# shibatch/rectdetect

Hardware: AMD Instinct MI355X
Metric: 1920x1080 frames/sec (higher is better)
Workload: dtype u8/i32/f32 (bit-exact integer + IEEE f32 stencil path)

## Files before the change

### include/rectdetect_hip.h

```cpp
#ifndef RECTDETECT_HIP_H
#define RECTDETECT_HIP_H
#include <stddef.h>
#include <stdint.h>
#if defined(__cplusplus)
extern "C" {
#endif

const char *rd_version(void);
int rd_device_count(void);
void rd_select_device(int ordinal);
int rd_device_pci_bus_id(int ordinal, char *buf, int len);

void *rd_device_alloc(size_t bytes);
void rd_device_free(void *dptr);
void *rd_host_alloc(size_t bytes);
void rd_host_free(void *p);
void rd_upload(void *dptr, const void *host, size_t bytes);
void rd_download(void *host, const void *dptr, size_t bytes);

typedef struct rd_detector rd_detector;

rd_detector *rd_detector_create(int device, int iw, int ih, int nslots, int nworkers);
void rd_detector_destroy(rd_detector *d);

rd_detector *rd_polyline_detector_create(int device, int iw, int ih, int nslots, int strength_thre, float minerror, int size_thre);
void *rd_detector_poll_segments(rd_detector *d, int32_t *ids_out);

void rd_release_cached_streams(int device);

#define RD_FRAME_HOST 0
#define RD_FRAME_DEVICE 1
#define RD_FRAME_HOST_PINNED 2
long rd_detector_enqueue(rd_detector *d, const void *frame, int ws, int on_device);

#define RD_PIX_BGR  0
#define RD_PIX_RGB  1
#define RD_PIX_BGRA 2
#define RD_PIX_RGBA 3
#define RD_PIX_NV12 4
#define RD_PIX_I420 5
long rd_detector_enqueue_planes(rd_detector *d, int format, const void *const planes[3], const int pitches[3], int on_device);

void *rd_detector_poll(rd_detector *d, double tanAOV);

void rd_detector_set_aperture(rd_detector *d, double tanAOV);

void rd_detector_drain(rd_detector *d);

int rd_detector_last_segments(rd_detector *d, void *dst, int max_records);

long rd_detector_counter(rd_detector *d, int which);


size_t rd_detector_debug_plane(rd_detector *d, const char *name, void *dst, size_t max_bytes);

void *rd_postprocess_planes(const void *segs, const int32_t *boundary, const int32_t *table, int iw, int ih, double tanAOV);
void rd_probe_pixels(float x0, float y0, float x1, float y1, int iw, int ih, int32_t *out);


void rd_rect_quads(const void *rects, int n, double *quads_out);
double rd_rect_aspect(const void *rect);
void rd_rectify_coefficients(const double quad[8], double coef[8], int *status);

typedef struct rd_rectifier rd_rectifier;
rd_rectifier *rd_rectifier_create(int device, int pw, int ph, int max_quads, int njobs);
void rd_rectifier_destroy(rd_rectifier *r);

long rd_rectifier_enqueue(rd_rectifier *r, int format, const void *const planes[3], const int pitches[3], int iw, int ih, int on_device,
                          const double *quads, int n, void *out, int out_kind);
int rd_rectifier_wait(rd_rectifier *r, uint8_t *status_out);
long rd_detector_rectify_polled(rd_detector *d, rd_rectifier *r, const double *quads, int n, void *out, int out_kind);

int rd_synth_num_quads(int iw, int ih);
void rd_synth_frame(uint8_t *bgr, int iw, int ih, int ws, uint64_t seed, int t, int noise);

#if defined(__cplusplus)
}
#endif
#endif
```

### rectdetect_amd/__init__.py

```python
import ctypes
import os

import numpy as np

_HERE = os.path.dirname(os.path.abspath(__file__))
LIB_PATH = os.environ.get("RD_LIB_PATH") or os.path.join(_HERE, "librectdetect_hip.so")

RECT_DTYPE = np.dtype([("c2", "<f8", (4, 2)), ("c3", "<f8", (4, 3)), ("value", "<f8"), ("status", "<u4"), ("_pad", "<u4")])
LS_DTYPE = np.dtype([("x0", "<f4"), ("y0", "<f4"), ("x1", "<f4"), ("y1", "<f4"), ("startIndex", "<i4"), ("endIndex", "<i4"),
                     ("leftPtr", "<i4"), ("rightPtr", "<i4"), ("startCount", "<i4"), ("endCount", "<i4"), ("maxDist", "<i4"),
                     ("polyid", "<i4"), ("npix", "<i4"), ("level", "<i4")])
assert RECT_DTYPE.itemsize == 176 and LS_DTYPE.itemsize == 56

PIX_BGR, PIX_RGB, PIX_BGRA, PIX_RGBA, PIX_NV12, PIX_I420 = range(6)
PIX_NAMES = {PIX_BGR: "BGR", PIX_RGB: "RGB", PIX_BGRA: "BGRA", PIX_RGBA: "RGBA", PIX_NV12: "NV12", PIX_I420: "I420"}

CL_MEM_READ_WRITE = 1 << 0
CL_MEM_COPY_HOST_PTR = 1 << 5
CL_TRUE = 1

_lib = None


def lib():
# ... 428 lines not shown
            raise ValueError("rd_rectifier_enqueue: invalid arguments (format %r, pitches %r, %dx%d, %d quads, out %r)" % (fmt, pitch, iw, ih, n, out))
        return r

    def wait(self):
        status = np.zeros(self.max_quads, np.uint8)
        n = lib().rd_rectifier_wait(self.h, status.ctypes.data)
        if n < 0:
            raise RuntimeError("rd_rectifier_wait: no job in flight")
        return status[:n].copy()

    def rectify(self, frame_bgr, quads):
        a = np.asarray(frame_bgr, dtype=np.uint8)
        q, n = _quads_arg(quads)
        nbytes = max(n, 1) * self.ph * self.pw * 3
        p = lib().rd_host_alloc(nbytes)
        try:
            self.enqueue(PIX_BGR, a, None, a.shape[1], a.shape[0], q, p, out_pinned=True)
            self.wait()
            return np.frombuffer((ctypes.c_uint8 * nbytes).from_address(p), np.uint8)[:n * self.ph * self.pw * 3].reshape(n, self.ph, self.pw, 3).copy()
        finally:
            lib().rd_host_free(p)

    def close(self):
        if self.h:
            lib().rd_rectifier_destroy(self.h)
            self.h = None


def postprocess_planes(segs, boundary, table, iw, ih, tan_aov):
    segs = np.ascontiguousarray(segs)
    boundary = np.ascontiguousarray(boundary, dtype=np.int32)
    table = np.ascontiguousarray(table, dtype=np.int32)
    return _take_rects(lib().rd_postprocess_planes(segs.ctypes.data, boundary.ctypes.data, table.ctypes.data, iw, ih, float(tan_aov)))
```

### rectdetect_amd/csrc/rd_api.hip

```cpp
#include "rd_internal.h"
#include "rd_kernels.h"
#include "rd_poly_scratch.h"
#include "rectdetect_hip.h"
#include <stdio.h>
#include <stdlib.h>
#include <string.h>
#include <pthread.h>
#include <time.h>
#include <sched.h>

extern "C" {
#include "vec234.h"
#include "oclimgutil.h"
#include "oclpolyline.h"
#include "oclrect.h"
#include "rd_post.h"
}

using rdrt::dptr;
using rdrt::stream;

static const char *rd_env(const char *name) { const char *v = getenv(name); return (v && *v) ? v : NULL; }
static int rd_env_int(const char *name, int dflt) { const char *v = rd_env(name); return v ? atoi(v) : dflt; }
#ifdef RD_TUNING
// ... 1387 lines not shown
      if (!strcmp(name, "strong") || !strcmp(name, "mergemask") || !strcmp(name, "junction")) {
        return bit_plane_as_ints(d, tab[i].p, !strcmp(name, "junction"), dst, max_bytes);
      }
      if (!strcmp(name, "mask0")) {
        const size_t n = N * 4 <= max_bytes ? N : max_bytes / 4;
        float *tmp = (float *)malloc(n ? n * 4 : 4);
        if (!tmp) exitf(-1, "rd_detector_debug_plane: out of memory\n");
        RD_HIP(hipMemcpy(tmp, s->nms, n * 4, hipMemcpyDeviceToHost));
        for (size_t k = 0; k < n; k++) ((int *)dst)[k] = tmp[k] > 0.0f ? 1 : 0;
        free(tmp);
        return n * 4;
      }
      if (!strcmp(name, "edge500")) {
        const size_t n = N * 4 <= max_bytes ? N : max_bytes / 4;
        int8_t *tmp = (int8_t *)malloc(n ? n : 1);
        RD_HIP(hipMemcpy(tmp, tab[i].p, n, hipMemcpyDeviceToHost));
        for (size_t k = 0; k < n; k++) ((int *)dst)[k] = tmp[k];
        free(tmp);
        return n * 4;
      }
      RD_HIP(hipMemcpy(dst, tab[i].p, b, hipMemcpyDeviceToHost));
      if (!strcmp(name, "strsum") && s->prev_in) {
        const size_t n = b / 4;
        int8_t *tmp = (int8_t *)malloc(n ? n : 1);
        RD_HIP(hipMemcpy(tmp, s->prev_in, n, hipMemcpyDeviceToHost));
        for (size_t k = 0; k < n; k++) ((int *)dst)[k] += tmp[k];
        free(tmp);
      }
      return b;
    }
  return 0;
}

rd_detector *rd_polyline_detector_create(int device, int iw, int ih, int nslots, int strength_thre, float minerror, int size_thre) {
  if (iw < 16 || ih < 16 || (long long)iw * ih >= (1ll << 25) || nslots < 1 || device < 0 || strength_thre < 0 || !(minerror > 0.0f) || size_thre < 0) return NULL;
  if (rd_device_count() <= 0) exitf(-1, "rd_polyline_detector_create: no HIP device available - this library has no CPU path\n");
  if (device >= rd_device_count()) return NULL;
  rd_detector *d = detector_new(RD_KIND_POLY, device, iw, ih, nslots, 0);
  d->p_thre = strength_thre; d->p_minerror = minerror; d->p_size = size_thre;
  d->handoff_rec = RD_POLY_HANDOFF_DEFAULT;
  { const int h = rd_env_int("RD_POLY_HANDOFF", 0); if (h >= 2) d->handoff_rec = h; }
  detector_slots(d, 4);
  return d;
}

void *rd_detector_poll_segments(rd_detector *d, int32_t *ids_out) {
  if (!d || d->magic != MAGIC_RECT) exitf(-1, "rd_detector_poll_segments: bad handle\n");
  if (d->kind != RD_KIND_POLY) exitf(-1, "rd_detector_poll_segments: this is a rectangle detector (rd_detector_create) - its results come from rd_detector_poll\n");
  if (d->next_poll >= d->next_enqueue) exitf(-1, "rd_detector_poll_segments: nothing enqueued\n");
  RD_HIP(hipSetDevice(d->device));
  const int si = (int)(d->next_poll % d->nslots);
  Slot *s = &d->slots[si];
  const size_t N = (size_t)d->N;
  if (s->pending_dense) group_launch(d, si / d->zb * d->zb);
  RD_HIP(hipEventSynchronize(s->watch_done));
  const bool over = s->poly_mode == 1 && s->h_pack[25] != 0;
  if (s->poly_mode == 1) { if (over) { if (++d->overflow_streak >= 2) d->poly_overflows = 1; } else d->overflow_streak = 0; }
  if (!s->st_redo) s->st_redo = make_redo_stream();
  if (over || (d->force_redo & 1)) {
    rdk::polyline(s->st_redo, s->frame, 1, d->N * 16, 0, d->p_minerror, d->p_size, d->iw, d->ih, 0);
    rdk::polyline_handoff(s->st_redo, s->frame, 1, d->handoff_rec);
    rdrt::check_launch("polyline frame, multi-launch repeat");
    RD_HIP(hipStreamSynchronize(s->st_redo));
    d->n_redo++;
  }
  const int n = s->h_pack[64];
// ... 71 lines not shown
```

### rectdetect_amd/csrc/rd_k_rect.hip

```cpp
#include <stdlib.h>
#include "rd_device.h"
#include "rd_kernels.h"
#include "rd_tidy_tile.h"
#include "rd_poly_scratch.h"
#include "rd_post_core.h"
#include <atomic>

namespace {

using namespace rd;

inline int cdiv(int a, int b) { return (a + b - 1) / b; }
const dim3 block2(64, 4);
inline dim3 grid2(int iw, int ih) { return dim3(cdiv(iw, 64), cdiv(ih, 4)); }
inline int ew_grid(int n) { int g = cdiv(n, 256 * 4); return g < 1 ? 1 : (g > 4096 ? 4096 : g); }

#define RD_XY const int x = blockIdx.x * 64 + threadIdx.x, y = blockIdx.y * 4 + rd_ty()

typedef unsigned long long u64;
__device__ __forceinline__ bitrow row_m1(const u64 *__restrict__ plane, int wpr, int y, int k, int ih) {
  if (y < 0 || y >= ih) return br(0, 0);
  const u64 *r = plane + (size_t)y * wpr + k;
  const u64 W = k > 0 ? r[-1] : 0ull, C = r[0], E = k + 1 < wpr ? r[1] : 0ull;
  return br((W >> 63) | (C << 1), (C >> 63) | (E << 1));
}
__global__ __launch_bounds__(256) void k_junction_bits(u64 *__restrict__ bits, const u64 *__restrict__ strong, int iw, int ih, int wpr, size_t zs) {
  RD_ZSHIFT(zs, bits, strong);
  const int t = blockIdx.x * 256 + threadIdx.x;
  if (t >= wpr * ih) return;
  const int y = t / wpr, k = t - y * wpr;
  const bitrow u = row_m1(strong, wpr, y - 1, k, ih), m = row_m1(strong, wpr, y, k, ih), d = row_m1(strong, wpr, y + 1, k, ih);
  bitrow ge1, ge2;
  br_count8(u, m, d, ge1, ge2);
  const bitrow in1 = (y >= 1 && y <= ih - 2) ? br_range(1 - 64 * k + 1, iw - 2 - 64 * k + 1) : br(0, 0);
  const bitrow any = m & in1 & ge1, end = any & ~ge2;
  bits[(size_t)t * 2] = (any.lo >> 1) | (any.hi << 63);
  bits[(size_t)t * 2 + 1] = (end.lo >> 1) | (end.hi << 63);
}

#ifndef BE_ROWS
#define BE_ROWS 32
#endif
#define BE_NR (BE_ROWS + 11)
__global__ __launch_bounds__(256) void k_blblur_extents(uint16_t *__restrict__ ext, const int8_t *__restrict__ edge, int iw, int ih, size_t zs) {
  RD_ZSHIFT(zs, ext, edge);
  typedef unsigned long long u64;
  __shared__ u64 EA[BE_NR + 1], EB[BE_NR + 1];
  __shared__ u64 HLa[BE_NR], HLb[BE_NR], HRa[BE_NR], HRb[BE_NR];
  __shared__ u64 VL[BE_NR], VR[BE_NR], VE[BE_NR];
  const int x0 = blockIdx.x * 64, y0 = blockIdx.y * BE_ROWS;
  const int tx = threadIdx.x, ty = rd_ty(), tid = ty * 64 + tx;
  {
    constexpr int IT = (BE_NR + 3) / 4;
    int8_t va[IT], vb[IT];
    bool oka[IT], okb[IT];
    const int xa = x0 - 8 + tx, xb = x0 + 56 + tx;
#pragma unroll
    for (int i = 0; i < IT; i++) {
      const int yy = y0 - 5 + ty + 4 * i;
      const bool rowin = ty + 4 * i < BE_NR && yy >= 0 && yy < ih;
      oka[i] = rowin && xa >= 0 && xa < iw;
      okb[i] = rowin && tx < 16 && xb < iw;
      va[i] = edge[oka[i] ? yy * iw + xa : 0];
      vb[i] = edge[okb[i] ? yy * iw + xb : 0];
    }
#pragma unroll
    for (int i = 0; i < IT; i++) {
      const int r = ty + 4 * i;
      const u64 ba = __ballot(oka[i] && va[i] != 0), bb = __ballot(okb[i] && vb[i] != 0);
      if (tx == 0 && r < BE_NR) { EA[r] = ba; EB[r] = bb; }
    }
  }
  if (tid == 0) { EA[BE_NR] = 0; EB[BE_NR] = 0; }
  __syncthreads();
  if (tid < BE_NR) {
    const int r = tid, yy = y0 - 5 + r;
    const u64 A = EA[r], B = EB[r], SA = EA[r + 1], SB = EB[r + 1];
    const u64 PA = A << 1, PB = (B << 1) | (A >> 63);
    const u64 NA = (A >> 1) | (B << 63), NB = B >> 1;
    u64 la = (A & ~PA) | (~A & PA & SA), lb = (B & ~PB) | (~B & PB & SB);
    u64 ra = ~A & NA, rb = ~B & NB;
    if (x0 == 0) { la &= ~(1ull << 8); la |= 0xffull; }
    const int fa = iw - x0 + 8, fb = iw - x0 - 56;
    if (fa < 64) ra |= ~0ull << fa;
    if (fb <= 0) rb = ~0ull; else if (fb < 64) rb |= ~0ull << fb;
    HLa[r] = la; HLb[r] = lb; HRa[r] = ra; HRb[r] = rb;
    const u64 Et = (A >> 8) | (B << 56), En = (A >> 9) | (B << 55);
    const u64 Ep = r > 0 ? (EA[r - 1] >> 8) | (EB[r - 1] << 56) : 0ull;
    const u64 Es = (SA >> 8) | (SB << 56);
    u64 vl = (Et & ~Ep) | (~Et & Ep & En);
    if (yy == 0) vl = 0;
    if (yy < 0) vl = ~0ull;
    u64 vr = ~Et & Es;
    if (yy >= ih) vr = ~0ull;
    VL[r] = vl; VR[r] = vr; VE[r] = Et;
  }
  __syncthreads();
  const int x = x0 + tx;
  if (x >= iw) return;
  for (int rr = ty; rr < BE_ROWS; rr += 4) {
    const int y = y0 + rr;
    if (y >= ih) break;
    const int r = rr + 5;
    const int sh = tx, rs = (64 - tx) & 63;
    const u64 keep = tx == 0 ? 0ull : ~0ull;
    const u64 we = (EA[r] >> sh) | ((EB[r] << rs) & keep);
    const u64 wl = (HLa[r] >> sh) | ((HLb[r] << rs) & keep);
    const u64 wr1 = (HRa[r] >> sh) | ((HRb[r] << rs) & keep);
    const bool oe = (we >> 8) & 1;
    const u64 wr = oe ? ~we : wr1;
    const unsigned tl = (unsigned)(wl >> 4) & 31u;
    const int nl = __clz((int)tl) - 27;
    const int nr = __ffs((int)(((unsigned)(wr >> 8) & 31u) | 32u)) - 1;
    unsigned tv = 0, uv = 32u;
#pragma unroll
    for (int d = 0; d < 5; d++) {
      tv |= (unsigned)((VL[r - d] >> tx) & 1ull) << (4 - d);
      const u64 w = oe ? ~VE[r + d] : VR[r + d];
      uv |= (unsigned)((w >> tx) & 1ull) << d;
    }
    const int nlv = __clz((int)tv) - 27, nrv = __ffs((int)uv) - 1;
    const int nrh = (nl | nr) ? nr : 1, nrvv = (nlv | nrv) ? nrv : 1;
    ext[y * iw + x] = (uint16_t)((unsigned)(nl | (nrh << 3)) | ((unsigned)(nlv | (nrvv << 3)) << 6));
  }
}

__device__ __forceinline__ unsigned div_small_m(unsigned s, unsigned m) { return __umul24(s, m) >> 19; }

#ifndef BQ_ROWS
#define BQ_ROWS 54
#endif
#define BQ_HR (BQ_ROWS + 8)
#define BQ_SW 73
static_assert(BQ_ROWS + 9 <= 64, "the column prefixes have 64 rows: the last output row reads prefix row BQ_ROWS + 8");
#ifndef BQ_WB
#define BQ_WB 2
#endif
__global__ __launch_bounds__(512) void k_blblur_pair(uint32_t *__restrict__ out, const uint16_t *__restrict__ ext, const uint32_t *__restrict__ in, int iw, int ih, size_t zs, int gdim) {
  const rd_tile rd_b = rd_block_tile(gdim);
  if (rd_b.x < 0) return;
  RD_ZSHIFTZ(rd_b.z, zs, out, ext, in);
  typedef unsigned long long u64;
  __shared__ u64 pl[BQ_HR * BQ_SW > 64 * 64 ? BQ_HR * BQ_SW : 64 * 64];
#ifndef BQ_PAD
#define BQ_PAD 0
#endif
  __shared__ u64 tot[8 * 64 + BQ_PAD];
  __shared__ unsigned rwt[16];
  const int tx = threadIdx.x, wv = rd_ty(), tid = wv * 64 + tx;
  const int x0 = rd_b.x * 64, y0 = rd_b.y * BQ_ROWS;
  const int x = x0 + tx;
  constexpr int NV = (BQ_ROWS + 7) / 8;
  unsigned eh[8], ev[NV];
  uint32_t q[9];
  const int sr = tid >> 3, sc = 64 + (tid & 7);
  const bool interior = x0 >= 4 && y0 >= 4 && x0 + 68 <= iw && y0 + BQ_ROWS + 4 <= ih;
// ... 116 lines not shown
      const unsigned e = ev[k0 + u] >> 6;
      const int nl = e & 7, nr = (e >> 3) & 7;
      const int r = wv + 8 * (k0 + u);
      const int c = ((r < BQ_ROWS ? r : 0) + 4) * 64 + tx;
      hi[u] = pl[c + nr * 64]; lo[u] = pl[c + (1 - nl) * 64]; c0[u] = pl[c]; c1[u] = pl[c + 64];
      rw[u] = rwt[nl + nr];
    }
#pragma unroll
    for (int u = 0; u < BQ_WB; u++) {
      if (k0 + u >= NV) continue;
      const int r = wv + 8 * (k0 + u);
      const int y = y0 + r;
      const u64 a = (hi[u] + c1[u]) - (lo[u] + c0[u]);
      const unsigned ax = (unsigned)a, ay = (unsigned)(a >> 32);
      if (r < BQ_ROWS && y < ih) atu(out, (unsigned)(y * iw + x)) = div_small_m(ax & 0xffffu, rw[u]) | (div_small_m(ax >> 16, rw[u]) << 12) | (div_small_m(ay, rw[u]) << 22);
    }
  }
}

__device__ __forceinline__ uint32_t quantize_plab(uint32_t v, int n0, int n1, int n2) {
  float L, a, b;
  unpack_lab(v, L, a, b);
  return pack_lab(roundf(L * n0) / (float)n0, roundf(a * n1) / (float)n1, roundf(b * n2) / (float)n2);
}

__device__ __attribute__((aligned(16))) uint16_t g_quant24[4096 + 1024];
__global__ void k_quant24_lut() {
  const int i = blockIdx.x * blockDim.x + threadIdx.x;
  if (i < 4096) g_quant24[i] = (uint16_t)(quantize_plab((uint32_t)i, 24, 24, 24) & 4095u);
  else if (i < 5120) g_quant24[i] = (uint16_t)((quantize_plab((uint32_t)(i - 4096) << 12, 24, 24, 24) >> 12) & 1023u);
}

#ifndef DS_ROWS
#define DS_ROWS 16
#endif
#define DS_P 66
template <int QN>
__global__ __launch_bounds__(256) void k_despeckle(uint32_t *__restrict__ out, const uint32_t *__restrict__ in, const float *__restrict__ edge, int iw, int ih, size_t zs, int gdim) {
  const rd_tile rd_b = rd_block_tile(gdim);
  if (rd_b.x < 0) return;
  RD_ZSHIFTZ(rd_b.z, zs, out, in, edge);
  constexpr int NC = (DS_ROWS + 2) * DS_P, IT = (NC + 255) / 256;
  __shared__ uint32_t tq[IT * 256];
  __shared__ uint8_t tf[IT * 256];
  __shared__ int list[64 * DS_ROWS];
  __shared__ int nlist;
  __shared__ uint32_t qlut[QN == 24 ? 2560 : 1];
  const int tx = threadIdx.x, tid = rd_ty() * 64 + tx;
  const int x0 = rd_b.x * 64, y0 = rd_b.y * DS_ROWS;
  if (tid == 0) nlist = 0;
  {
    uint32_t v[IT];
    float e[IT];
    bool ok[IT];
#pragma unroll
    for (int i = 0; i < IT; i++) {
      const int t = tid + 256 * i;
      const int xx = x0 - 1 + t % DS_P, yy = y0 - 1 + t / DS_P;
      ok[i] = t < NC && xx >= 0 && xx < iw && yy >= 0 && yy < ih;
      const int a = ok[i] ? yy * iw + xx : 0;
      v[i] = in[a];
      e[i] = edge[a];
    }
    if (QN == 24) {
      uint32_t w[10];
#pragma unroll
      for (int i = 0; i < 10; i++) w[i] = ((const uint32_t *)g_quant24)[tid + 256 * i];
#pragma unroll
      for (int i = 0; i < 10; i++) qlut[tid + 256 * i] = w[i];
      __syncthreads();
    }
#pragma unroll
    for (int i = 0; i < IT; i++) {
      const int t = tid + 256 * i;
      uint32_t qv = v[i];
      if (QN == 24) {
        const uint16_t *q16 = (const uint16_t *)qlut;
        qv = (uint32_t)q16[qv & 4095u] | ((uint32_t)q16[4096 + ((qv >> 12) & 1023u)] << 12) | ((uint32_t)q16[4096 + (qv >> 22)] << 22);
      } else if (QN > 0) qv = quantize_plab(qv, QN, QN, QN);
      tq[t] = ok[i] ? qv : 0u;
      tf[t] = ok[i] ? (uint8_t)((!(e[i] < 1e-6f) ? 1 : 0) | (e[i] >= 1e-6f ? 2 : 0)) : (uint8_t)4;
    }
  }
  __syncthreads();
  for (int r = rd_ty(); r < DS_ROWS; r += 4) {
    const int x = x0 + tx, y = y0 + r;
    const int i = (r + 1) * DS_P + tx + 1;
    bool hot = false;
    if (x < iw && y < ih) {
      hot = tf[i] & 1;
      if (!hot) out[y * iw + x] = tq[i];
    }
    const unsigned long long m = __ballot(hot);
    if (m) {
      const int leader = __ffsll((long long)m) - 1;
      int o = 0;
      if (tx == leader) o = atomicAdd(&nlist, __popcll(m));
      o = __shfl(o, leader);
      if (hot) list[o + __popcll(m & ((1ull << tx) - 1))] = i;
    }
  }
  __syncthreads();
  const int n = nlist;
  for (int j = tid; j < n; j += 256) {
    const int i = list[j];
    uint32_t r = tq[i];
    float dist = 1e+10f, l0, a0, b0;
    unpack_lab(r, l0, a0, b0);
#pragma unroll
    for (int k = 0; k < 9; k++) {
      const int q = i + (k / 3 - 1) * DS_P + k % 3 - 1;
      if (tf[q] & 6) continue;
      float l1, a1, b1;
      const uint32_t v = tq[q];
      unpack_lab(v, l1, a1, b1);
      const float dx = l1 - l0, dy = a1 - a0, dz = b1 - b0;
      const float d = sqrtf(dx * dx + dy * dy + dz * dz);
      if (d < dist) { r = v; dist = d; }
    }
    out[(y0 + i / DS_P - 1) * iw + x0 + i % DS_P - 1] = r;
  }
}

template <int DX>
__device__ __forceinline__ unsigned long long mm_shift(unsigned long long w0, unsigned long long w1, unsigned long long w2) {
  if (DX == 0) return w1;
  if (DX > 0) return (w1 >> DX) | (w2 << (64 - DX));
  return (w1 << -DX) | (w0 >> (64 + DX));
}
template <int DY, int LO, int HI, int DX = -8>
__device__ __forceinline__ unsigned long long mm_row(unsigned long long w0, unsigned long long w1, unsigned long long w2) {
  unsigned long long r = 0;
  if (DX * DX + DY * DY >= LO && DX * DX + DY * DY < HI) r = mm_shift<DX>(w0, w1, w2);
  if constexpr (DX < 8) r |= mm_row<DY, LO, HI, DX + 1>(w0, w1, w2);
  return r;
}
template <int DY>
__device__ __forceinline__ void mm_rows(const unsigned long long *sb, int r, unsigned long long &A, unsigned long long &B, unsigned long long &C) {
  const unsigned long long *row = sb + (r + 8 + DY) * 6;
  const unsigned long long a0 = row[0], a1 = row[1], a2 = row[2], e0 = row[3], e1 = row[4], e2 = row[5];
  constexpr int ADY = DY < 0 ? -DY : DY;
  if (ADY * ADY < 36) A |= mm_row<ADY, 16, 36>(a0, a1, a2);
  if (ADY * ADY < 64) B |= mm_row<ADY, 0, 64>(e0, e1, e2);
  if (ADY * ADY < 16) C |= mm_row<ADY, 0, 16>(a0 & ~e0, a1 & ~e1, a2 & ~e2);
  if constexpr (DY < 8) mm_rows<DY + 1>(sb, r, A, B, C);
}

#define MM_ROWS 64
__global__ __launch_bounds__(256) void k_mm_gather(unsigned long long *__restrict__ out, const unsigned long long *__restrict__ bits, int iw, int ih, int wpr, size_t zs) {
  RD_ZSHIFT(zs, out, bits);
  __shared__ unsigned long long sb[(MM_ROWS + 16) * 6];
  const int k = blockIdx.x;
  const int y0 = blockIdx.y * MM_ROWS;
// ... 600 lines not shown
          if (st[k] < tag) {
            const int i = atomicAdd(&nloc, 1);
            if (i < D2A_CAP) loc[i] = q[k]; else list_out[atomicAdd(count_out, 1)] = q[k];
          }
      }
      __syncthreads();
      if (nloc + 256 * 12 > D2A_CAP) d2_flush(list_out, count_out, loc, nloc, base, tid);
    }
  }
  if (list_out != nullptr) d2_flush(list_out, count_out, loc, nloc, base, tid);
}

__global__ __launch_bounds__(256) void k_despeckle2_active(int *__restrict__ nxt, const int *__restrict__ cur, const int *__restrict__ list, const int *__restrict__ count,
                                                            int *__restrict__ list_out, int *count_out, int *count_zero, int *work_trace, int *__restrict__ stamp, int tag,
                                                            const int *__restrict__ old, const int *__restrict__ size, int thre, int iw, int ih) {
  __shared__ int loc[D2A_CAP];
  __shared__ int nloc, base;
  d2_active_rounds(nxt, cur, list, count, list_out, count_out, count_zero, work_trace, stamp, tag, old, size, thre, iw, ih, blockIdx.x, gridDim.x, loc, nloc, base);
}

#define AB_TW 64
#ifndef AB_TH
#define AB_TH 64
#endif
#ifndef AB_HK
#define AB_HK 16
#endif
#define AB_LW (AB_TW + 2 * AB_HK + 2)
#define AB_LH (AB_TH + AB_HK + 2)
#define AB_NC (AB_LW * AB_LH)
#ifndef AB_NT
#define AB_NT 512
#endif
#define AB_R 4
#define AB_INEXACT 0x40000000u
typedef unsigned long long ab_word;
__device__ __forceinline__ ab_word ab_pack(int lab, unsigned t) { return ((ab_word)t << 32) | (unsigned)lab; }
__device__ __forceinline__ int ab_lab(ab_word w) { return (int)(unsigned)w; }
__device__ __forceinline__ unsigned ab_t(ab_word w) { return (unsigned)(w >> 32); }

#define AB_REC 12
__device__ __forceinline__ void ab_record(int *__restrict__ rec, int p, int rl, unsigned rs, const ab_word *cell, int c, int iw, int gx0, int gy0) {
  const int d[4] = { -AB_LW - 1, -AB_LW, -AB_LW + 1, -1 };
  int v[AB_REC];
  v[0] = p; v[1] = rl; v[2] = (int)rs; v[11] = 0;
#pragma unroll
  for (int j = 0; j < 4; j++) {
    const int cj = c + d[j];
    const ab_word w = cell[cj];
    const bool undecided = (ab_t(w) & AB_INEXACT) != 0;
    v[3 + j] = undecided ? -((gy0 + cj / AB_LW) * iw + gx0 + cj % AB_LW) - 2 : ab_lab(w);
    v[7 + j] = undecided ? 0 : (int)ab_t(w);
  }
#pragma unroll
  for (int q = 0; q < AB_REC; q += 4) *(int4 *)(rec + q) = make_int4(v[q], v[q + 1], v[q + 2], v[q + 3]);
}

__global__ __launch_bounds__(AB_NT) void k_absorb_tile(int *__restrict__ out, int *__restrict__ list, int reccap, int *count, const int *__restrict__ old, const int *__restrict__ size,
                                                       int thre, int iw, int ih, size_t zs, int gdim) {
  const rd_tile rd_b = rd_block_tile(gdim);
  if (rd_b.x < 0) return;
  RD_ZSHIFTZ(rd_b.z, zs, out, list, count, old, size);
  __shared__ ab_word cell[AB_NC];
  __shared__ unsigned short slist[AB_NT * AB_R];
  __shared__ unsigned short rlist[AB_TW * AB_TH];
  __shared__ int nsmall, nres, base;
  const int tid = threadIdx.x;
  if (tid == 0) { nsmall = 0; nres = 0; }
  const int gx0 = rd_b.x * AB_TW - AB_HK - 1, gy0 = rd_b.y * AB_TH - AB_HK - 1;
  {
    constexpr int IT = (AB_NC + AB_NT - 1) / AB_NT;
    int l[IT], sz[IT];
// ... 18 lines not shown
      const bool inner = cx >= 1 && cx <= AB_LW - 2 && cy >= 1 && cy <= AB_LH - 2;
      cell[t] = ab_pack(in[i] ? l[i] : -1, in[i] ? ((unsigned)sz[i] | (small ? AB_INEXACT : 0u)) : 0u);
      if (small && inner) {
        const int k = atomicAdd(&nsmall, 1);
        if (k < AB_NT * AB_R) slist[k] = (unsigned short)t;
      }
    }
  }
  __syncthreads();
  const int ns = nsmall;
  int c[AB_R], rl[AB_R], slot[AB_R];
  unsigned rs[AB_R];
  bool open[AB_R];
#pragma unroll
  for (int k = 0; k < AB_R; k++) { open[k] = false; slot[k] = -1; c[k] = AB_LW + 1; rl[k] = 0; rs[k] = 0; }
  const bool owned = ns > 0 && ns <= AB_NT * AB_R;
  if (owned) {
#pragma unroll
    for (int k = 0; k < AB_R; k++) {
      const int i = tid + k * AB_NT;
      open[k] = i < ns;
      c[k] = open[k] ? slist[i] : AB_LW + 1;
      const ab_word w0 = cell[c[k]], w1 = cell[c[k] + 1], w2 = cell[c[k] + AB_LW - 1], w3 = cell[c[k] + AB_LW], w4 = cell[c[k] + AB_LW + 1];
      rl[k] = ab_lab(w0); rs[k] = ab_t(w0) & ~AB_INEXACT;
      unsigned t;
      t = ab_t(w1) & ~AB_INEXACT; if (t > rs[k]) { rs[k] = t; rl[k] = ab_lab(w1); }
      t = ab_t(w2) & ~AB_INEXACT; if (t > rs[k]) { rs[k] = t; rl[k] = ab_lab(w2); }
      t = ab_t(w3) & ~AB_INEXACT; if (t > rs[k]) { rs[k] = t; rl[k] = ab_lab(w3); }
      t = ab_t(w4) & ~AB_INEXACT; if (t > rs[k]) { rs[k] = t; rl[k] = ab_lab(w4); }
    }
    __syncthreads();
    for (int round = 0; round < AB_HK + 8; round++) {
      bool progress = false;
#pragma unroll
      for (int k = 0; k < AB_R; k++) {
        if (!open[k]) continue;
        const ab_word p0 = cell[c[k] - AB_LW - 1], p1 = cell[c[k] - AB_LW], p2 = cell[c[k] - AB_LW + 1], p3 = cell[c[k] - 1];
        if ((ab_t(p0) | ab_t(p1) | ab_t(p2) | ab_t(p3)) & AB_INEXACT) continue;
        unsigned bs = 0; int bl = rl[k];
        if (ab_t(p0) > bs) { bs = ab_t(p0); bl = ab_lab(p0); }
        if (ab_t(p1) > bs) { bs = ab_t(p1); bl = ab_lab(p1); }
        if (ab_t(p2) > bs) { bs = ab_t(p2); bl = ab_lab(p2); }
        if (ab_t(p3) > bs) { bs = ab_t(p3); bl = ab_lab(p3); }
        if (rs[k] > bs) { bs = rs[k]; bl = rl[k]; }
        cell[c[k]] = ab_pack(bl, bs);
        open[k] = false;
        progress = true;
      }
      if (!__syncthreads_or(progress)) break;
    }
#pragma unroll
    for (int k = 0; k < AB_R; k++) {
      const int cx = c[k] % AB_LW - (AB_HK + 1), cy = c[k] / AB_LW - (AB_HK + 1);
      if (open[k] && cx >= 0 && cx < AB_TW && cy >= 0 && cy < AB_TH) slot[k] = atomicAdd(&nres, 1);
    }
  }
  const int tx = tid & 63, x = rd_b.x * AB_TW + tx;
  for (int r = tid >> 6; r < AB_TH; r += AB_NT / 64) {
    const int y = rd_b.y * AB_TH + r;
    if (x >= iw || y >= ih) continue;
    const int ci = (r + AB_HK + 1) * AB_LW + tx + AB_HK + 1;
    const ab_word w = cell[ci];
    if (!(ab_t(w) & AB_INEXACT)) out[(unsigned)(y * iw + x)] = ab_lab(w);
    else if (!owned) rlist[atomicAdd(&nres, 1)] = (unsigned short)ci;
  }
  __syncthreads();
  const int nr = nres;
  if (nr == 0) return;
  if (tid == 0) base = atomicAdd(count, nr);
  __syncthreads();
  if (owned) {
#pragma unroll
    for (int k = 0; k < AB_R; k++) {
      if (slot[k] < 0) continue;
      const int p = (gy0 + c[k] / AB_LW) * iw + gx0 + c[k] % AB_LW, at = base + slot[k];
      out[(unsigned)p] = -at - 2;
      if (at < reccap) ab_record(list + (size_t)at * AB_REC, p, rl[k], rs[k], cell, c[k], iw, gx0, gy0);
    }
  } else {
    for (int i = tid; i < nr; i += AB_NT) {
// ... 590 lines not shown
```

Baseline: 2916.

## Run several wavefront-local resolve passes per barrier round in despeckle absorb

The absorb kernel's iterative resolve loop now repeats up to AB_PASSES inner passes inside each block-wide barrier round. It uses relaxed atomic loads and stores so lanes can see neighbours resolved in the same round, and stops early when no lane in the wavefront moves. The aim is to cut the number of __syncthreads_or rounds needed to propagate labels through the dependency chains. In exchange it adds atomic memory traffic and possible extra work for wavefronts that spin without progress. A debug entry point, rd_debug_absorb, with a Python wrapper is also added for testing the absorb stage.

New measurement: 2933 (median of 6 runs). No clear change (+0.6%).

```diff
diff --git a/include/rectdetect_hip.h b/include/rectdetect_hip.h
--- a/include/rectdetect_hip.h
+++ b/include/rectdetect_hip.h
@@ -53,6 +53,7 @@
 
 
 size_t rd_detector_debug_plane(rd_detector *d, const char *name, void *dst, size_t max_bytes);
+int rd_debug_absorb(int device, const int *labels, const int *size_init, int iw, int ih, int nz, int thre, int *region_out, int *rsize_out, int *status_out);
 
 void *rd_postprocess_planes(const void *segs, const int32_t *boundary, const int32_t *table, int iw, int ih, double tanAOV);
 void rd_probe_pixels(float x0, float y0, float x1, float y1, int iw, int ih, int32_t *out);
diff --git a/rectdetect_amd/__init__.py b/rectdetect_amd/__init__.py
--- a/rectdetect_amd/__init__.py
+++ b/rectdetect_amd/__init__.py
@@ -484,3 +484,28 @@
     boundary = np.ascontiguousarray(boundary, dtype=np.int32)
     table = np.ascontiguousarray(table, dtype=np.int32)
     return _take_rects(lib().rd_postprocess_planes(segs.ctypes.data, boundary.ctypes.data, table.ctypes.data, iw, ih, float(tan_aov)))
+
+
+def debug_absorb(labels, size_init=None, thre=16, device=0):
+    L = lib()
+    fn = L.rd_debug_absorb
+    fn.restype, fn.argtypes = ctypes.c_int, [ctypes.c_int, ctypes.c_void_p, ctypes.c_void_p] + [ctypes.c_int] * 4 + [ctypes.c_void_p] * 3
+    lab = np.ascontiguousarray(labels, dtype=np.int32)
+    planes = lab.reshape((-1,) + lab.shape[-2:])
+    nz, ih, iw = planes.shape
+    dl, ds = L.rd_device_alloc(planes.nbytes), None
+    try:
+        L.rd_upload(dl, planes.ctypes.data, planes.nbytes)
+        if size_init is not None:
+            s0 = np.ascontiguousarray(size_init, dtype=np.int32)
+            assert s0.shape == lab.shape
+            ds = L.rd_device_alloc(s0.nbytes)
+            L.rd_upload(ds, s0.ctypes.data, s0.nbytes)
+        region, rsize, status = np.empty_like(planes), np.empty_like(planes), np.zeros((nz, 4), np.int32)
+        if fn(device, dl, ds, iw, ih, nz, thre, region.ctypes.data, rsize.ctypes.data, status.ctypes.data) != 0:
+            raise ValueError("rd_debug_absorb: arguments out of range")
+    finally:
+        L.rd_device_free(dl)
+        if ds:
+            L.rd_device_free(ds)
+    return region.reshape(lab.shape), rsize.reshape(lab.shape), status
diff --git a/rectdetect_amd/csrc/rd_api.hip b/rectdetect_amd/csrc/rd_api.hip
--- a/rectdetect_amd/csrc/rd_api.hip
+++ b/rectdetect_amd/csrc/rd_api.hip
@@ -1443,6 +1443,40 @@
   return 0;
 }
 
+int rd_debug_absorb(int device, const int *labels, const int *size_init, int iw, int ih, int nz, int thre, int *region_out, int *rsize_out, int *status_out) {
+  if (!labels || !region_out || !rsize_out || !status_out || iw < 1 || ih < 1 || (long long)iw * ih >= (1ll << 25) || nz < 1 || nz > 8 || device < 0 || device >= rd_device_count()) return -1;
+  RD_HIP(hipSetDevice(device));
+  const size_t N = (size_t)iw * ih;
+  const size_t o_lab = 0, o_size = N, o_out = 2 * N, o_d2 = 3 * N, o_status = o_d2 + RD_D2_SCRATCH_INTS(N), per = (o_status + 16 + 63) & ~(size_t)63, zs = per * sizeof(int);
+  int *base = NULL;
+  hipStream_t st;
+  RD_HIP(hipMalloc((void **)&base, zs * nz));
+  RD_HIP(hipStreamCreateWithFlags(&st, hipStreamNonBlocking));
+  RD_HIP(hipMemsetAsync(base, 0, zs * nz, st));
+  for (int z = 0; z < nz; z++) {
+    RD_HIP(hipMemcpyAsync(base + z * per + o_lab, labels + z * N, N * sizeof(int), hipMemcpyDeviceToDevice, st));
+    if (size_init) RD_HIP(hipMemcpyAsync(base + z * per + o_size, size_init + z * N, N * sizeof(int), hipMemcpyDeviceToDevice, st));
+  }
+  rdk::region_size(st, base + o_size, base + o_lab, (int)N, base + o_d2 + N, 0, nz, zs);
+  rdk::despeckle2(st, base + o_out, base + o_lab, base + o_d2, base + o_size, thre, iw, ih, 1, base + o_status, nz, zs);
+  RD_HIP(hipStreamSynchronize(st));
+  for (int z = 0; z < nz; z++) {
+    int *f = base + z * per;
+    RD_HIP(hipMemcpy(status_out + 4 * z, f + o_status, 3 * sizeof(int), hipMemcpyDeviceToHost));
+    status_out[4 * z + 3] = 0;
+    if (status_out[4 * z] != 0) {
+      rdk::despeckle2_slow(st, f + o_out, f + o_lab, f + o_d2, f + o_size, thre, iw, ih);
+      RD_HIP(hipStreamSynchronize(st));
+      status_out[4 * z + 3] = 1;
+    }
+    RD_HIP(hipMemcpy(region_out + z * N, f + o_out, N * sizeof(int), hipMemcpyDeviceToHost));
+    RD_HIP(hipMemcpy(rsize_out + z * N, f + o_size, N * sizeof(int), hipMemcpyDeviceToHost));
+  }
+  RD_HIP(hipStreamDestroy(st));
+  RD_HIP(hipFree(base));
+  return 0;
+}
+
 rd_detector *rd_polyline_detector_create(int device, int iw, int ih, int nslots, int strength_thre, float minerror, int size_thre) {
   if (iw < 16 || ih < 16 || (long long)iw * ih >= (1ll << 25) || nslots < 1 || device < 0 || strength_thre < 0 || !(minerror > 0.0f) || size_thre < 0) return NULL;
   if (rd_device_count() <= 0) exitf(-1, "rd_polyline_detector_create: no HIP device available - this library has no CPU path\n");
diff --git a/rectdetect_amd/csrc/rd_k_rect.hip b/rectdetect_amd/csrc/rd_k_rect.hip
--- a/rectdetect_amd/csrc/rd_k_rect.hip
+++ b/rectdetect_amd/csrc/rd_k_rect.hip
@@ -1057,12 +1057,16 @@
 #ifndef AB_NT
 #define AB_NT 512
 #endif
+#ifndef AB_PASSES
+#define AB_PASSES 8
+#endif
 #define AB_R 4
 #define AB_INEXACT 0x40000000u
 typedef unsigned long long ab_word;
 __device__ __forceinline__ ab_word ab_pack(int lab, unsigned t) { return ((ab_word)t << 32) | (unsigned)lab; }
 __device__ __forceinline__ int ab_lab(ab_word w) { return (int)(unsigned)w; }
 __device__ __forceinline__ unsigned ab_t(ab_word w) { return (unsigned)(w >> 32); }
+__device__ __forceinline__ ab_word ab_load(const ab_word *p) { return __atomic_load_n(p, __ATOMIC_RELAXED); }
 
 #define AB_REC 12
 __device__ __forceinline__ void ab_record(int *__restrict__ rec, int p, int rl, unsigned rs, const ab_word *cell, int c, int iw, int gx0, int gy0) {
@@ -1147,20 +1151,26 @@
     __syncthreads();
     for (int round = 0; round < AB_HK + 8; round++) {
       bool progress = false;
-#pragma unroll
-      for (int k = 0; k < AB_R; k++) {
-        if (!open[k]) continue;
-        const ab_word p0 = cell[c[k] - AB_LW - 1], p1 = cell[c[k] - AB_LW], p2 = cell[c[k] - AB_LW + 1], p3 = cell[c[k] - 1];
-        if ((ab_t(p0) | ab_t(p1) | ab_t(p2) | ab_t(p3)) & AB_INEXACT) continue;
-        unsigned bs = 0; int bl = rl[k];
-        if (ab_t(p0) > bs) { bs = ab_t(p0); bl = ab_lab(p0); }
-        if (ab_t(p1) > bs) { bs = ab_t(p1); bl = ab_lab(p1); }
-        if (ab_t(p2) > bs) { bs = ab_t(p2); bl = ab_lab(p2); }
-        if (ab_t(p3) > bs) { bs = ab_t(p3); bl = ab_lab(p3); }
-        if (rs[k] > bs) { bs = rs[k]; bl = rl[k]; }
-        cell[c[k]] = ab_pack(bl, bs);
-        open[k] = false;
-        progress = true;
+#pragma unroll 1
+      for (int pass = 0; pass < AB_PASSES; pass++) {
+        bool moved = false;
+#pragma unroll
+        for (int k = 0; k < AB_R; k++) {
+          if (!open[k]) continue;
+          const ab_word p0 = ab_load(&cell[c[k] - AB_LW - 1]), p1 = ab_load(&cell[c[k] - AB_LW]), p2 = ab_load(&cell[c[k] - AB_LW + 1]), p3 = ab_load(&cell[c[k] - 1]);
+          if ((ab_t(p0) | ab_t(p1) | ab_t(p2) | ab_t(p3)) & AB_INEXACT) continue;
+          unsigned bs = 0; int bl = rl[k];
+          if (ab_t(p0) > bs) { bs = ab_t(p0); bl = ab_lab(p0); }
+          if (ab_t(p1) > bs) { bs = ab_t(p1); bl = ab_lab(p1); }
+          if (ab_t(p2) > bs) { bs = ab_t(p2); bl = ab_lab(p2); }
+          if (ab_t(p3) > bs) { bs = ab_t(p3); bl = ab_lab(p3); }
+          if (rs[k] > bs) { bs = rs[k]; bl = rl[k]; }
+          __atomic_store_n(&cell[c[k]], ab_pack(bl, bs), __ATOMIC_RELAXED);
+          open[k] = false;
+          moved = true;
+        }
+        progress = progress || moved;
+        if (!__any(moved)) break;
       }
       if (!__syncthreads_or(progress)) break;
     }
```

## Restructure blblur extents and despeckle tile loading with precomputed bit-plane counts

Applied to the files above, without the earlier changes.

The extents kernel now precomputes per-row, per-column run-length counts for all five horizontal and vertical offsets as bit-planes. Two waves do this work, and the results are packed into shared memory. Each output thread then assembles its 12-bit code with rotates instead of per-pixel shift, clz and ffs chains. The despeckle kernel switches to a taller row tile (DS_ROWS 30) with one row-per-wave load layout, separate halo columns, per-wave hot lists with no shared atomics, 16-bit list entries, and simplified flags. This trades extra per-block setup work and changed occupancy for less redundant per-pixel work and fewer scattered loads.

New measurement: 2906 before, 2950 after, median of 6. 1.5% higher.

```diff
diff --git a/rectdetect_amd/csrc/rd_k_rect.hip b/rectdetect_amd/csrc/rd_k_rect.hip
--- a/rectdetect_amd/csrc/rd_k_rect.hip
+++ b/rectdetect_amd/csrc/rd_k_rect.hip
@@ -42,39 +42,45 @@
 #define BE_ROWS 32
 #endif
 #define BE_NR (BE_ROWS + 11)
+static_assert(BE_ROWS % 4 == 0 && BE_ROWS <= 64, "rows by four waves; one lane per tile row");
+__device__ __forceinline__ unsigned long long be_cols(unsigned long long A, unsigned long long B, int d) { return (A >> (8 + d)) | (B << (56 - d)); }
+__device__ __forceinline__ void be_count(const unsigned long long (&stop)[5], unsigned long long &b0, unsigned long long &b1, unsigned long long &b2, unsigned long long &any) {
+  const unsigned long long c1 = ~stop[0], c2 = c1 & ~stop[1], c3 = c2 & ~stop[2], c4 = c3 & ~stop[3], c5 = c4 & ~stop[4];
+  b0 = (c1 & ~c2) | (c3 & ~c4) | c5; b1 = c2 & ~c4; b2 = c4; any = c1;
+}
+union be_word { uint32_t w; uint16_t h[2]; };
 __global__ __launch_bounds__(256) void k_blblur_extents(uint16_t *__restrict__ ext, const int8_t *__restrict__ edge, int iw, int ih, size_t zs) {
   RD_ZSHIFT(zs, ext, edge);
   typedef unsigned long long u64;
-  __shared__ u64 EA[BE_NR + 1], EB[BE_NR + 1];
-  __shared__ u64 HLa[BE_NR], HLb[BE_NR], HRa[BE_NR], HRb[BE_NR];
-  __shared__ u64 VL[BE_NR], VR[BE_NR], VE[BE_NR];
+  __shared__ u64 EA[BE_NR], EB[BE_NR];
+  __shared__ __attribute__((aligned(16))) be_word PW[BE_ROWS][4][6];
   const int x0 = blockIdx.x * 64, y0 = blockIdx.y * BE_ROWS;
-  const int tx = threadIdx.x, ty = rd_ty(), tid = ty * 64 + tx;
+  const int tx = threadIdx.x, ty = rd_ty();
   {
     constexpr int IT = (BE_NR + 3) / 4;
     int8_t va[IT], vb[IT];
-    bool oka[IT], okb[IT];
     const int xa = x0 - 8 + tx, xb = x0 + 56 + tx;
+    const bool cola = xa >= 0 && xa < iw, colb = tx < 16 && xb < iw;
+    const unsigned ca = cola ? (unsigned)xa : 0u, cb = colb ? (unsigned)xb : 0u;
 #pragma unroll
     for (int i = 0; i < IT; i++) {
       const int yy = y0 - 5 + ty + 4 * i;
       const bool rowin = ty + 4 * i < BE_NR && yy >= 0 && yy < ih;
-      oka[i] = rowin && xa >= 0 && xa < iw;
-      okb[i] = rowin && tx < 16 && xb < iw;
-      va[i] = edge[oka[i] ? yy * iw + xa : 0];
-      vb[i] = edge[okb[i] ? yy * iw + xb : 0];
+      const unsigned rb = rowin ? (unsigned)(yy * iw) : 0u;
+      va[i] = atu(edge, rb + ca);
+      vb[i] = atu(edge, rb + cb);
     }
 #pragma unroll
     for (int i = 0; i < IT; i++) {
-      const int r = ty + 4 * i;
-      const u64 ba = __ballot(oka[i] && va[i] != 0), bb = __ballot(okb[i] && vb[i] != 0);
+      const int r = ty + 4 * i, yy = y0 - 5 + r;
+      const bool rowin = r < BE_NR && yy >= 0 && yy < ih;
+      const u64 ba = __builtin_amdgcn_ballot_w64(rowin && cola && va[i] != 0), bb = __builtin_amdgcn_ballot_w64(rowin && colb && vb[i] != 0);
       if (tx == 0 && r < BE_NR) { EA[r] = ba; EB[r] = bb; }
     }
   }
-  if (tid == 0) { EA[BE_NR] = 0; EB[BE_NR] = 0; }
-  __syncthreads();
-  if (tid < BE_NR) {
-    const int r = tid, yy = y0 - 5 + r;
+  __syncthreads();
+  if (ty == 0 && tx < BE_ROWS) {
+    const int r = tx + 5;
     const u64 A = EA[r], B = EB[r], SA = EA[r + 1], SB = EB[r + 1];
     const u64 PA = A << 1, PB = (B << 1) | (A >> 63);
     const u64 NA = (A >> 1) | (B << 63), NB = B >> 1;
@@ -84,44 +90,64 @@
     const int fa = iw - x0 + 8, fb = iw - x0 - 56;
     if (fa < 64) ra |= ~0ull << fa;
     if (fb <= 0) rb = ~0ull; else if (fb < 64) rb |= ~0ull << fb;
-    HLa[r] = la; HLb[r] = lb; HRa[r] = ra; HRb[r] = rb;
-    const u64 Et = (A >> 8) | (B << 56), En = (A >> 9) | (B << 55);
-    const u64 Ep = r > 0 ? (EA[r - 1] >> 8) | (EB[r - 1] << 56) : 0ull;
-    const u64 Es = (SA >> 8) | (SB << 56);
-    u64 vl = (Et & ~Ep) | (~Et & Ep & En);
-    if (yy == 0) vl = 0;
-    if (yy < 0) vl = ~0ull;
-    u64 vr = ~Et & Es;
-    if (yy >= ih) vr = ~0ull;
-    VL[r] = vl; VR[r] = vr; VE[r] = Et;
+    const u64 Et = be_cols(A, B, 0);
+    u64 sl[5], sr[5];
+#pragma unroll
+    for (int d = 0; d < 5; d++) {
+      sl[d] = be_cols(la, lb, -d);
+      sr[d] = (Et & ~be_cols(A, B, d)) | (~Et & be_cols(ra, rb, d));
+    }
+    u64 p[6], anyl, anyr;
+    be_count(sl, p[0], p[1], p[2], anyl);
+    be_count(sr, p[3], p[4], p[5], anyr);
+    p[3] |= ~anyl & ~anyr;
+#pragma unroll
+    for (int k = 0; k < 6; k++)
+#pragma unroll
+      for (int q = 0; q < 4; q++) PW[tx][q][k].h[0] = (uint16_t)(p[k] >> (16 * q));
+  }
+  if (ty == 1 && tx < BE_ROWS) {
+    const int r = tx + 5, yy = y0 + tx;
+    u64 E[11];
+#pragma unroll
+    for (int k = 0; k < 11; k++) E[k] = be_cols(EA[r - 5 + k], EB[r - 5 + k], 0);
+    u64 sl[5], sr[5];
+#pragma unroll
+    for (int d = 0; d < 5; d++) {
+      const u64 Ec = E[5 - d], Ep = E[4 - d], En = be_cols(EA[r - d], EB[r - d], 1);
+      u64 vl = (Ec & ~Ep) | (~Ec & Ep & En);
+      if (yy - d == 0) vl = 0;
+      if (yy - d < 0) vl = ~0ull;
+      sl[d] = vl;
+      u64 vr = (E[5] & ~E[5 + d]) | (~E[5] & ~E[5 + d] & E[6 + d]);
+      if (yy + d >= ih) vr = ~0ull;
+      sr[d] = vr;
+    }
+    u64 p[6], anyl, anyr;
+    be_count(sl, p[0], p[1], p[2], anyl);
+    be_count(sr, p[3], p[4], p[5], anyr);
+    p[3] |= ~anyl & ~anyr;
+#pragma unroll
+    for (int k = 0; k < 6; k++)
+#pragma unroll
+      for (int q = 0; q < 4; q++) PW[tx][q][k].h[1] = (uint16_t)(p[k] >> (16 * q));
   }
   __syncthreads();
   const int x = x0 + tx;
   if (x >= iw) return;
-  for (int rr = ty; rr < BE_ROWS; rr += 4) {
-    const int y = y0 + rr;
-    if (y >= ih) break;
-    const int r = rr + 5;
-    const int sh = tx, rs = (64 - tx) & 63;
-    const u64 keep = tx == 0 ? 0ull : ~0ull;
-    const u64 we = (EA[r] >> sh) | ((EB[r] << rs) & keep);
-    const u64 wl = (HLa[r] >> sh) | ((HLb[r] << rs) & keep);
-    const u64 wr1 = (HRa[r] >> sh) | ((HRb[r] << rs) & keep);
-    const bool oe = (we >> 8) & 1;
-    const u64 wr = oe ? ~we : wr1;
-    const unsigned tl = (unsigned)(wl >> 4) & 31u;
-    const int nl = __clz((int)tl) - 27;
-    const int nr = __ffs((int)(((unsigned)(wr >> 8) & 31u) | 32u)) - 1;
-    unsigned tv = 0, uv = 32u;
-#pragma unroll
-    for (int d = 0; d < 5; d++) {
-      tv |= (unsigned)((VL[r - d] >> tx) & 1ull) << (4 - d);
-      const u64 w = oe ? ~VE[r + d] : VR[r + d];
-      uv |= (unsigned)((w >> tx) & 1ull) << d;
-    }
-    const int nlv = __clz((int)tv) - 27, nrv = __ffs((int)uv) - 1;
-    const int nrh = (nl | nr) ? nr : 1, nrvv = (nlv | nrv) ? nrv : 1;
-    ext[y * iw + x] = (uint16_t)((unsigned)(nl | (nrh << 3)) | ((unsigned)(nlv | (nrvv << 3)) << 6));
+  const int piece = tx >> 4, turn = tx & 15;
+  uint32_t w[BE_ROWS / 4][6];
+#pragma unroll
+  for (int i = 0; i < BE_ROWS / 4; i++)
+#pragma unroll
+    for (int k = 0; k < 6; k++) w[i][k] = PW[ty + 4 * i][piece][k].w;
+#pragma unroll
+  for (int i = 0; i < BE_ROWS / 4; i++) {
+    const int y = y0 + ty + 4 * i;
+    uint32_t t = 0;
+#pragma unroll
+    for (int k = 0; k < 6; k++) t |= __builtin_rotateright32(w[i][k], (unsigned)(turn - k) & 31u) & (0x10001u << k);
+    if (y < ih) atu(ext, (unsigned)(y * iw + x)) = (uint16_t)((t & 63u) | ((t >> 16) << 6));
   }
 }
 
@@ -304,93 +330,105 @@
 }
 
 #ifndef DS_ROWS
-#define DS_ROWS 16
+#define DS_ROWS 30
 #endif
 #define DS_P 66
+#define DS_R (DS_ROWS + 2)
+#define DS_RW (DS_R / 4)
+static_assert(DS_R % 4 == 0 && 2 * DS_R <= 256 && DS_R <= 64, "rows by four waves; one halo cell per thread; a list entry is row << 6 | column in 16 bits");
 template <int QN>
 __global__ __launch_bounds__(256) void k_despeckle(uint32_t *__restrict__ out, const uint32_t *__restrict__ in, const float *__restrict__ edge, int iw, int ih, size_t zs, int gdim) {
   const rd_tile rd_b = rd_block_tile(gdim);
   if (rd_b.x < 0) return;
   RD_ZSHIFTZ(rd_b.z, zs, out, in, edge);
-  constexpr int NC = (DS_ROWS + 2) * DS_P, IT = (NC + 255) / 256;
-  __shared__ uint32_t tq[IT * 256];
-  __shared__ uint8_t tf[IT * 256];
-  __shared__ int list[64 * DS_ROWS];
-  __shared__ int nlist;
+  __shared__ uint32_t tq[DS_R * DS_P];
+  __shared__ uint8_t tf[DS_R * DS_P];
+  __shared__ uint16_t list[4][64 * DS_RW];
+  __shared__ int nlist[4];
   __shared__ uint32_t qlut[QN == 24 ? 2560 : 1];
-  const int tx = threadIdx.x, tid = rd_ty() * 64 + tx;
+  const int tx = threadIdx.x, wv = rd_ty(), tid = wv * 64 + tx;
   const int x0 = rd_b.x * 64, y0 = rd_b.y * DS_ROWS;
-  if (tid == 0) nlist = 0;
+  const bool colin = x0 + tx < iw;
+  const unsigned cx = (unsigned)(x0 + (colin ? tx : 0));
+  uint32_t v[DS_RW + 1];
+  float e[DS_RW + 1];
+#pragma unroll
+  for (int k = 0; k < DS_RW; k++) {
+    const int y = y0 - 1 + wv + 4 * k, yc = y < 0 ? 0 : (y >= ih ? ih - 1 : y);
+    const unsigned a = (unsigned)(yc * iw) + cx;
+    v[k] = atu(in, a);
+    e[k] = atu(edge, a);
+  }
+  const int hs = tid >> 1, hc = (tid & 1) * (DS_P - 1);
+  const int hx = x0 - 1 + hc, hy = y0 - 1 + hs;
+  const bool hok = hs < DS_R && hx >= 0 && hx < iw && hy >= 0 && hy < ih;
   {
-    uint32_t v[IT];
-    float e[IT];
-    bool ok[IT];
-#pragma unroll
-    for (int i = 0; i < IT; i++) {
-      const int t = tid + 256 * i;
-      const int xx = x0 - 1 + t % DS_P, yy = y0 - 1 + t / DS_P;
-      ok[i] = t < NC && xx >= 0 && xx < iw && yy >= 0 && yy < ih;
-      const int a = ok[i] ? yy * iw + xx : 0;
-      v[i] = in[a];
-      e[i] = edge[a];
-    }
+    const unsigned a = hok ? (unsigned)(hy * iw + hx) : 0u;
+    v[DS_RW] = atu(in, a);
+    e[DS_RW] = atu(edge, a);
+  }
+  if (QN == 24) {
+    uint32_t w[10];
+#pragma unroll
+    for (int i = 0; i < 10; i++) w[i] = atu((const uint32_t *)g_quant24, (unsigned)(tid + 256 * i));
+#pragma unroll
+    for (int i = 0; i < 10; i++) qlut[tid + 256 * i] = w[i];
+    __syncthreads();
+  }
+  auto quant = [&](uint32_t c) -> uint32_t {
     if (QN == 24) {
-      uint32_t w[10];
-#pragma unroll
-      for (int i = 0; i < 10; i++) w[i] = ((const uint32_t *)g_quant24)[tid + 256 * i];
-#pragma unroll
-      for (int i = 0; i < 10; i++) qlut[tid + 256 * i] = w[i];
-      __syncthreads();
-    }
-#pragma unroll
-    for (int i = 0; i < IT; i++) {
-      const int t = tid + 256 * i;
-      uint32_t qv = v[i];
-      if (QN == 24) {
-        const uint16_t *q16 = (const uint16_t *)qlut;
-        qv = (uint32_t)q16[qv & 4095u] | ((uint32_t)q16[4096 + ((qv >> 12) & 1023u)] << 12) | ((uint32_t)q16[4096 + (qv >> 22)] << 22);
-      } else if (QN > 0) qv = quantize_plab(qv, QN, QN, QN);
-      tq[t] = ok[i] ? qv : 0u;
-      tf[t] = ok[i] ? (uint8_t)((!(e[i] < 1e-6f) ? 1 : 0) | (e[i] >= 1e-6f ? 2 : 0)) : (uint8_t)4;
-    }
-  }
-  __syncthreads();
-  for (int r = rd_ty(); r < DS_ROWS; r += 4) {
-    const int x = x0 + tx, y = y0 + r;
-    const int i = (r + 1) * DS_P + tx + 1;
-    bool hot = false;
-    if (x < iw && y < ih) {
-      hot = tf[i] & 1;
-      if (!hot) out[y * iw + x] = tq[i];
-    }
-    const unsigned long long m = __ballot(hot);
+      const uint16_t *q16 = (const uint16_t *)qlut;
+      return (uint32_t)q16[c & 4095u] | ((uint32_t)q16[4096 + ((c >> 12) & 1023u)] << 12) | ((uint32_t)q16[4096 + (c >> 22)] << 22);
+    }
+    return QN > 0 ? quantize_plab(c, QN, QN, QN) : c;
+  };
+#pragma unroll
+  for (int k = 0; k <= DS_RW; k++) v[k] = quant(v[k]);
+  int nhot = 0;
+#pragma unroll
+  for (int k = 0; k < DS_RW; k++) {
+    const int s = wv + 4 * k, y = y0 - 1 + s;
+    const bool ok = colin && y >= 0 && y < ih, mine = ok && s >= 1 && s <= DS_ROWS;
+    const uint32_t qv = v[k];
+    const bool hot = !(e[k] < 1e-6f), skip = e[k] >= 1e-6f;
+    const int i = s * DS_P + tx + 1;
+    tq[i] = qv;
+    tf[i] = ok && !skip ? 0 : 1;
+    if (mine && !hot) atu(out, (unsigned)(y * iw + x0 + tx)) = qv;
+    const unsigned long long m = __builtin_amdgcn_ballot_w64(mine && hot);
     if (m) {
-      const int leader = __ffsll((long long)m) - 1;
-      int o = 0;
-      if (tx == leader) o = atomicAdd(&nlist, __popcll(m));
-      o = __shfl(o, leader);
-      if (hot) list[o + __popcll(m & ((1ull << tx) - 1))] = i;
-    }
-  }
-  __syncthreads();
-  const int n = nlist;
+      if (mine && hot) list[wv][nhot + (int)__builtin_amdgcn_mbcnt_hi((unsigned)(m >> 32), __builtin_amdgcn_mbcnt_lo((unsigned)m, 0u))] = (uint16_t)((s << 6) | tx);
+      nhot += __popcll(m);
+    }
+  }
+  if (hs < DS_R) {
+    const int i = hs * DS_P + hc;
+    tq[i] = v[DS_RW];
+    tf[i] = hok && !(e[DS_RW] >= 1e-6f) ? 0 : 1;
+  }
+  if (tx == 0) nlist[wv] = nhot;
+  __syncthreads();
+  const int n1 = nlist[0], n2 = n1 + nlist[1], n3 = n2 + nlist[2], n = n3 + nlist[3];
   for (int j = tid; j < n; j += 256) {
-    const int i = list[j];
+    const int w = (j >= n1) + (j >= n2) + (j >= n3);
+    const int en = list[w][j - (w == 0 ? 0 : (w == 1 ? n1 : (w == 2 ? n2 : n3)))];
+    const int s = en >> 6, c = en & 63;
+    const int i = s * DS_P + c + 1;
     uint32_t r = tq[i];
     float dist = 1e+10f, l0, a0, b0;
     unpack_lab(r, l0, a0, b0);
 #pragma unroll
     for (int k = 0; k < 9; k++) {
       const int q = i + (k / 3 - 1) * DS_P + k % 3 - 1;
-      if (tf[q] & 6) continue;
+      if (tf[q]) continue;
       float l1, a1, b1;
-      const uint32_t v = tq[q];
-      unpack_lab(v, l1, a1, b1);
+      const uint32_t v1 = tq[q];
+      unpack_lab(v1, l1, a1, b1);
       const float dx = l1 - l0, dy = a1 - a0, dz = b1 - b0;
       const float d = sqrtf(dx * dx + dy * dy + dz * dz);
-      if (d < dist) { r = v; dist = d; }
-    }
-    out[(y0 + i / DS_P - 1) * iw + x0 + i % DS_P - 1] = r;
+      if (d < dist) { r = v1; dist = d; }
+    }
+    atu(out, (unsigned)((y0 + s - 1) * iw + x0 + c)) = r;
   }
 }
 
```
